# SenseBrain/JPD-SE

Hardware: AMD Instinct MI355X
Metric: training images/sec at 1024x512 (G+D+VGG step) (higher is better)
Workload: dtype bf16; 1 GPU; JPD-SE train step 1024x512, netG=global ngf=64 (39-ch input), num_D=2, VGG19+feat+L1, Adam x2, batch 4/GPU; global_batch=4, parallelism=dp1

## Files before the change

jpd-se_amd/csrc/conv_dispatch_fwd.h:

```cpp
#pragma once

namespace jpdse {

struct FwdCall {
  const jpdse_conv_desc* d; const ConvPlan& p;
  const void* x; const void* pack; const float* bias; void* y; void* ws; hipStream_t s;
  float* mom; void* pool; bool* pooled;
};

static int fwd_thin_in_rows(const FwdCall& c) {
  ThinInArgs g = {};
  g.DY = reinterpret_cast<const bf16_t*>(c.x);
  g.P = reinterpret_cast<const bf16_t*>(c.pack);
  g.DX = reinterpret_cast<bf16_t*>(c.y);
  g.bias = c.bias;
  g.act = c.d->act; g.slope = c.d->slope;
  g.N = c.d->N; g.H = c.d->H; g.W = c.d->W; g.OH = c.p.OH; g.OW = c.p.OW;
  g.py = g.px = 1;
  return launch_thin_in_rows<3, false>(g, c.s);
}

static int thin_fwd_slots(const ConvPlan& p, const ThinFwdGeom& tg) {
  return (p.OH % tg.TH == 0 && p.OW % tg.TW == 0) ? (p.OH / tg.TH) * (p.OW / tg.TW) : 0;
}
// ... 37 lines not shown
  HeadFwdArgs h = {};
  h.X = reinterpret_cast<const bf16_t*>(c.x);
  h.Wp = reinterpret_cast<const bf16_t*>(c.pack);
  h.bias = c.bias;
  h.Y = reinterpret_cast<bf16_t*>(c.y);
  h.N = d->N; h.H = d->H; h.W = d->W; h.OH = p.OH; h.OW = p.OW;
  h.K = d->K; h.Ks_out = p.Ks;
  h.R = d->R; h.S = d->S; h.pad = d->pad;
  h.reflect = d->pad_mode == JPDSE_PAD_REFLECT;
  h.act = d->act; h.slope = d->slope;
  h.tiles_w = (p.OW + 63) / 64;
  h.tiles_h = (p.OH + kHeadTH - 1) / kHeadTH;
  if (route == FwdRoute::head_rows) return p.Cs == 64 ? launch_head_rows<7>(h, c.s) : launch_head_rows<7, 32>(h, c.s);
  return p.Cs == 64 ? launch_head_fwd<64>(h, c.s) : launch_head_fwd<32>(h, c.s);
}

static int fwd_tapsum(const FwdCall& c) {
  const jpdse_conv_desc* d = c.d;
  const ConvPlan& p = c.p;
  const int cols = d->K * d->R * d->S, zs = (cols + 7) / 8 * 8;
  FastArgs f = {};
  f.X = reinterpret_cast<const bf16_t*>(c.x);
  f.B = reinterpret_cast<const bf16_t*>(c.pack);
  f.M = d->N * d->H * d->W; f.OH = f.IH = d->H; f.OW = f.IW = d->W;
  f.Cs = p.Cs; f.R = f.S = 1; f.sy = f.sx = 1;
  f.Kout = f.b_rows = cols; f.Ks = zs;
  f.act = JPDSE_ACT_NONE;
  f.splits = 1; f.no_finish = 1; f.partial = reinterpret_cast<float*>(c.ws);
  if (int rc = launch_fast(f, c.s)) return rc;
  const long long total = (long long)d->N * p.OH * p.OW * p.Ks;
  hipLaunchKernelGGL(tapsum_kernel, dim3((unsigned)((total + 255) / 256)), dim3(256), 0, c.s, f.partial, c.bias,
                     reinterpret_cast<bf16_t*>(c.y), d->N, d->H, d->W, p.OH, p.OW, d->K, p.Ks, d->R, d->S, d->pad,
                     d->pad_mode == JPDSE_PAD_REFLECT ? 1 : 0, zs, d->act, d->slope, total);
  return check_launch("tapsum_kernel");
}

static ConvView fwd_view(const FwdCall& c) {
  ConvView v = view_fwd(c.d, c.p, c.x, c.pack, c.bias, c.y);
  v.mom = c.mom;
  return v;
}
static float* splitk_slabs(const ConvPlan& p, void* ws) { return reinterpret_cast<float*>(reinterpret_cast<char*>(ws) + p.splitk_off); }

static int fwd_halo(const FwdCall& c) {
  HaloArgs h = to_halo(fwd_view(c));
  if (c.pool != nullptr && c.mom == nullptr && c.pooled != nullptr) {
    h.pool = reinterpret_cast<bf16_t*>(c.pool);
    *c.pooled = true;
  }
  return c.p.Ks > 64 ? launch_halo_cfg<2>(h, c.s) : launch_halo_cfg<1>(h, c.s);
}

static int fwd_fast(const FwdCall& c) {
  FastArgs f = to_fast(fwd_view(c));
  f.splits = splitk_for(f.M, c.p.Ks, c.d->R * c.d->S * c.p.Cs / 64);
  f.partial = splitk_slabs(c.p, c.ws);
  return launch_fast(f, c.s);
}

template <typename T>
static int fwd_gemm(const FwdCall& c, bool toep) {
  const jpdse_conv_desc* d = c.d;
  const ConvPlan& p = c.p;
  if (int rc = launch_pad<T>(c.x, c.ws, d->N, d->H, d->W, p.Cs, d->pad, d->pad, d->pad, d->pad, d->pad_mode, c.s)) return rc;
  const int px = toep ? 4 : 1, Lk = toep ? p.Lk_toep : p.Lk_fwd;
  GemmFwdArgs a = {};
  a.A = c.ws;
  a.B = toep ? reinterpret_cast<const char*>(c.pack) + p.fwd_pack_plain_bytes : c.pack;
  a.bias = c.bias;
  a.Y = c.y;
  a.OH = p.OH; a.OW = p.OW / px; a.M = d->N * a.OH * a.OW;
  a.Kout = toep ? 32 : d->K; a.Ks = a.b_rows = toep ? 32 : p.Ks;
  a.R = d->R; a.cpr = Lk / p.BKE; a.b_row_stride = (long long)d->R * Lk;
  a.in_sn = (long long)p.Hp * p.Wp * p.Cs; a.in_sr = (long long)p.Wp * p.Cs;
  a.in_sh = (long long)d->stride * p.Wp * p.Cs;
  a.in_sw = (long long)px * d->stride * p.Cs;
  a.out_sn = (long long)p.OH * p.OW * p.Ks; a.out_sh = (long long)p.OW * p.Ks; a.out_sw = (long long)px * p.Ks;
  a.act = d->act; a.slope = d->slope;
  if (toep) {
    a.col_mod = 8;
    a.k_real = d->K;
  } else {
    a.partial = splitk_slabs(p, c.ws);
    a.partial_cap = p.splitk_bytes;
  }
  return launch_fwd<T>(a, c.s);
}

template <typename T>
static int conv_fwd_t(const jpdse_conv_desc* d, const ConvPlan& p, const void* x, const void* pack,
                      const float* bias, void* y, void* ws, hipStream_t s, float* mom = nullptr, void* pool = nullptr,
                      bool* pooled = nullptr) {
  const FwdCall c = {d, p, x, pack, bias, y, ws, s, mom, pool, pooled};
  const FwdRoute route = select_fwd(d, p, {mom != nullptr, pool != nullptr});
  if constexpr (sizeof(T) == 2) {
    switch (route) {
      case FwdRoute::thin_in_rows: return fwd_thin_in_rows(c);
      case FwdRoute::thin_rows:
      case FwdRoute::thin_fwd: return fwd_thin(c, route);
      case FwdRoute::head_rows:
      case FwdRoute::head_fwd: return fwd_head(c, route);
      case FwdRoute::tapsum: return fwd_tapsum(c);
      case FwdRoute::rows: return launch_rows(to_rows(fwd_view(c)), d->stride, s);
      case FwdRoute::taps4: return launch_taps4(fwd_view(c), ws, s);
      case FwdRoute::taps9: return launch_taps9(fwd_view(c), splitk_slabs(p, ws), s);
      case FwdRoute::halo: return fwd_halo(c);
// ... 21 lines not shown
```

jpd-se_amd/csrc/conv_gemm.hip:

```cpp
#include "common.h"

#include <vector>


namespace jpdse {

struct GemmFwdArgs {
  const void* A;
  const void* B;
  const float* bias;
  void* Y;
  int M, OH, OW;
  int Kout, Ks;
  int R, cpr;
  int b_rows;
  long long b_row_stride;
  long long in_sn, in_sh, in_sw, in_sr, in_base;
  long long out_sn, out_sh, out_sw, out_base;
  int act;
  float slope;
  int col_mod, k_real;
  int splits;
  float* partial;
  size_t partial_cap;
// ... 93 lines not shown
  if (threadIdx.x == 0) reinterpret_cast<volatile int*>(occ_smem)[0] = (int)blockIdx.x;
  const unsigned long long t0 = __builtin_amdgcn_s_memrealtime();
  while (true) {
    const int r = __hip_atomic_load(release, __ATOMIC_RELAXED, __HIP_MEMORY_SCOPE_SYSTEM);
    if (r != 0) break;
    if (__builtin_amdgcn_s_memrealtime() - t0 > max_ticks) break;
    __builtin_amdgcn_s_sleep(127);
  }
}

int jpdse_debug_occupy_cus(int32_t blocks, const int32_t* release_flag, int32_t max_ms, void* stream) {
  JPDSE_REQUIRE(blocks > 0 && blocks <= 128 && release_flag != nullptr && max_ms > 0 && max_ms <= 20000,
                "debug_occupy_cus: blocks in 1..128, a flag, max_ms in 1..20000");
  constexpr int lds = 160 * 1024;
  if (int rc = opt_in_lds<&occupy_cus_kernel>("occupy_cus", lds)) return rc;
  hipLaunchKernelGGL(occupy_cus_kernel, dim3(blocks), dim3(256), lds, as_stream(stream), release_flag,
                     (unsigned long long)max_ms * 100000ULL);
  return check_launch("occupy_cus_kernel");
}

int jpdse_debug_set_fast_path(int32_t enable) {
  if (enable == 19 || enable == 28 || enable == 42 || enable == 43 || (enable >= 50 && enable <= 54) || enable == 56 || enable == 61 ||
      (enable >= 100 && enable <= 199) || (enable >= 201 && enable <= 203) || (enable >= 210 && enable <= 225))
    return set_error(JPDSE_EINVAL, "debug_set_fast_path: mode %d is retired (its code path was removed; see include/jpdse_dev.h)", (int)enable);
  g_fast_enabled = enable != 0;
  g_halo_enabled = enable != 3;
  g_moments_fused = enable != 32 && enable != 6;
  g_ring_virt = enable != 40 && enable != 6;
  g_thin1_enabled = enable != 41 && enable != 6;
  g_taps9_enabled = enable != 38 && enable != 6;
  g_taps4_enabled = enable != 36 && enable != 6;
  g_taps_enabled = enable != 35 && enable != 6;
  g_rows_enabled = enable != 29 && enable != 3;
  g_wgrad_nine_enabled = enable != 4;
  g_wgrad_taps_enabled = enable != 12;
  g_ring_enabled = enable != 7 && enable != 3;
  g_merge_min_kt = enable == 9 ? 16 : 4;
  g_norm_fused = enable != 27;
  g_merge_min_tiles = enable == 26 ? 384 : 64;
  g_fast_small = enable == 10 ? 0 : 20;
  g_halo_xcd = enable == 15 ? 1 : (enable == 16 ? 2 : (enable == 17 ? 3 : 0));
  g_halo_single = enable != 8;
  g_head_fwd_enabled = enable != 14 && enable != 6;
  g_thin_fwd_enabled = enable != 18;
  g_tapsum_enabled = enable != 13;
  g_thin_out_fast = enable != 13;
  g_toep_enabled = enable != 5;
  g_wgrad_nine32_enabled = enable != 55;
  g_head_rows32 = enable != 57;
  g_halo_xcd_auto = enable != 60;
  g_fast_fill = enable != 59;
  g_wgrad_taps_xcd = enable == 58;
  g_generic_splitk = enable != 48;
  g_splitk_enabled = enable != 6;
  return JPDSE_OK;
}

int jpdse_debug_conv_route(const jpdse_conv_desc* d, int32_t flags, int32_t out[3]) {
  if (int rc = validate(d)) return rc;
  JPDSE_REQUIRE(out != nullptr && (flags & ~0x7f) == 0, "debug_conv_route: null output or unknown flag bits");
  ConvPlan p;
  make_plan(d, &p);
  out[0] = (int32_t)select_fwd(d, p, {(flags & 1) != 0, (flags & 2) != 0});
  out[1] = (int32_t)select_dgrad(d, p, {(flags & 4) != 0, (flags & 8) != 0, (flags & 4) != 0 && (flags & 16) != 0, (flags & 32) != 0, (flags & 64) != 0});
  out[2] = (int32_t)select_wgrad(d, p);
  return JPDSE_OK;
}

const char* jpdse_debug_route_name(int32_t direction, int32_t route) {
  if (route < 0) return nullptr;
  if (direction == 0 && route <= (int)FwdRoute::generic) return route_name((FwdRoute)route);
  if (direction == 1 && route <= (int)DgradRoute::generic) return route_name((DgradRoute)route);
  if (direction == 2 && route <= (int)WgradRoute::generic) return route_name((WgradRoute)route);
  return nullptr;
}
#endif

int jpdse_prof_select(int32_t enable, int32_t Ks, int64_t kdim, int32_t max_launches) {
  g_prof.on = false;
  g_prof.used = 0;
  if (!enable) return JPDSE_OK;
  JPDSE_REQUIRE(Ks > 0 && kdim > 0 && max_launches > 0, "prof_select: bad selection");
  while ((int)g_prof.ev.size() < 2 * max_launches) {
    hipEvent_t e;
    if (hipEventCreate(&e) != hipSuccess) return set_error(JPDSE_ELAUNCH, "prof_select: hipEventCreate failed");
    g_prof.ev.push_back(e);
  }
  g_prof.flops.assign(max_launches, 0.0);
  g_prof.cls.assign(max_launches, 0);
  g_prof.Ks = Ks;
  g_prof.kdim = kdim;
  g_prof.on = true;
  return JPDSE_OK;
}

static int prof_sum(int cls, double* total_ms, double* total_flops, int64_t* launches) {
  double ms = 0.0, fl = 0.0;
  int64_t n = 0;
  for (int i = 0; i < g_prof.used; ++i) {
    if (g_prof.cls[i] != cls) continue;
    if (hipEventSynchronize(g_prof.ev[2 * i + 1]) != hipSuccess)
      return set_error(JPDSE_ELAUNCH, "prof_collect: hipEventSynchronize failed");
    float t = 0.f;
    if (hipEventElapsedTime(&t, g_prof.ev[2 * i], g_prof.ev[2 * i + 1]) != hipSuccess)
      return set_error(JPDSE_ELAUNCH, "prof_collect: hipEventElapsedTime failed");
    ms += t;
// ... 343 lines not shown
```

jpd-se_amd/csrc/conv_launch.h:

```cpp
#pragma once

namespace jpdse {

struct GemmProf {
  bool on = false;
  int Ks = 0;
  long long kdim = 0;
  int used = 0;
  std::vector<hipEvent_t> ev;
  std::vector<double> flops;
  std::vector<int> cls;
};
static GemmProf g_prof;
static int check_tile_grid(const char* who, int N, int OH, int OW, int th, int tw, int Cs_in, long long in_elems, long long out_elems) {
  if (N <= 0 || OH <= 0 || OW <= 0 || OH % th != 0 || OW % tw != 0)
    return set_error(JPDSE_EINVAL, "%s: output grid %d x %d x %d does not tile into %d x %d patches", who, N, OH, OW, th, tw);
  if (Cs_in <= 0 || Cs_in % 64 != 0) return set_error(JPDSE_EINVAL, "%s: %d input channels (a multiple of 64 is required)", who, Cs_in);
  if (in_elems >= (1LL << 31) || out_elems >= (1LL << 40))
    return set_error(JPDSE_EINVAL, "%s: tensor too large for the kernel's offsets (%lld input elements)", who, in_elems);
  return JPDSE_OK;
}

template <auto Kernel>
static int opt_in_lds(const char* who, int bytes) {
// ... 543 lines not shown
  a.mask = v.mask;
  a.prog[0].B[0] = v.B;
  a.prog[0].ktot[0] = v.ktot;
  a.prog[0].out_base[0] = v.out_base;
  for (int r = 0; r < v.R; ++r)
    for (int c = 0; c < v.S; ++c) {
      a.prog[0].tap_off[r * v.S + c] = r * patch_w + c;
      a.prog[0].tap_koff[r * v.S + c] = r * v.tap_r + c * v.tap_s;
    }
  return a;
}

static int launch_taps4(const ConvView& v, void* ws, hipStream_t s) {
  const int OHc = v.OH / 8 * 8, OWc = v.OW / 32 * 32;
  TapsArgs a = to_taps(v, 35);
  a.OH = OHc;
  a.OW = OWc;
  const int bn = v.Ks_out % 128 == 0 ? 128 : 64;
  a.nblk0 = v.N * (OHc / 8) * (OWc / 32) * ((v.Ks_out + bn - 1) / bn);
  if (int rc = bn == 128 ? launch_taps4_cfg<2>(a, a.nblk0, s) : launch_taps4_cfg<1>(a, a.nblk0, s)) return rc;
  const int k_tiles = 16 * v.Cin_s / 64;
  const int sp = taps4_fringe_splits(v.N, v.OH, v.OW, v.Ks_out, k_tiles);
  if (sp == 0) return JPDSE_OK;
  FastBatch fb = {};
  float* slab = reinterpret_cast<float*>(ws);
  const int rect[2][4] = {{OHc, 0, v.OH - OHc, v.OW}, {0, OWc, OHc, v.OW - OWc}};
  for (int q = 0; q < 2; ++q) {
    const int oh0 = rect[q][0], ow0 = rect[q][1], rows = rect[q][2], cols = rect[q][3];
    if (rows <= 0 || cols <= 0) continue;
    FastArgs g = to_fast(v);
    g.M = v.N * rows * cols;
    g.OH = rows;
    g.OW = cols;
    g.py = v.py - oh0;
    g.px = v.px - ow0;
    g.out_base = v.out_base + oh0 * v.out_sh + ow0 * v.out_sw;
    g.splits = sp;
    g.no_finish = 1;
    g.partial = slab;
    g.b_stride = v.ktot;
    g.b_tap_r = v.tap_r;
    g.b_tap_s = v.tap_s;
    slab += (size_t)sp * g.M * v.Ks_out;
    fb.p[fb.n++] = g;
  }
  if (int rc = launch_fast_batch(fb, s)) return rc;
  for (int q = 0; q < fb.n; ++q) {
    const long long total_vec = (long long)fb.p[q].M * (fb.p[q].Ks / 8);
    hipLaunchKernelGGL(splitk_finish_kernel, dim3(ew_blocks(total_vec)), dim3(256), 0, s, fb.p[q], total_vec);
  }
  return check_launch("taps4 fringe finish");
}

static int taps9_splits(int N, int OH, int OW, int Cin_s, int Ks_out) {
  const int sp = splitk_for(N * OH * OW, Ks_out, 9 * Cin_s / 64);
  const int cc = Cin_s / 64;
  return sp > cc / 2 ? (cc / 2 > 0 ? cc / 2 : 1) : sp;
}

template <int TN, bool VIRT = false>
static int launch_taps9_cfg(const TapsArgs& a, int total, hipStream_t s) {
  constexpr int PH = 10, PW = 34;
  constexpr int lds = 2 * ((PH * PW + 7) / 8) * 1024 + 3 * (2 * TN * 32) * 128;
  if (int rc = opt_in_lds<&gemm_taps_kernel<TN, 9, 0, 0, 0, 2, PH, PW, VIRT>>("gemm_taps(3x3)", lds)) return rc;
  if (int rc = check_tile_grid("gemm_taps(3x3)", a.N, a.OH, a.OW, 8, 32, a.Cs, (long long)a.N * a.IH * a.IW * a.Cs,
                               (long long)a.N * a.OH * a.OW * a.Ks)) return rc;
  const int sp = a.splits > 1 ? a.splits : 1;
  if (total != sp * a.N * (a.OH / 8) * (a.OW / 32) * ((a.Ks + 2 * TN * 32 - 1) / (2 * TN * 32)) || (sp > 1 && a.partial == nullptr))
    return set_error(JPDSE_EINVAL, "gemm_taps(3x3): %d blocks do not match the tile grid x %d splits", total, sp);
  if (VIRT && (a.V == nullptr || a.py != 1 || a.px != 1 || a.IH != a.OH || a.IW != a.OW || a.OH < 16 || a.reflect))
    return set_error(JPDSE_EINVAL, "gemm_taps(3x3): folded-frame form needs a frame, pad 1, equal grids, >= 16 rows");
  hipLaunchKernelGGL((gemm_taps_kernel<TN, 9, 0, 0, 0, 2, PH, PW, VIRT>), dim3(total), dim3(512), lds, s, a);
  return check_launch("gemm_taps_kernel(3x3)");
}

static int launch_taps9(const ConvView& v, float* slabs, hipStream_t s) {
  TapsArgs a = to_taps(v, 34);
  a.reflect = v.reflect;
  a.V = v.frame;
  const int bn = v.Ks_out % 128 == 0 ? 128 : 64;
  const int tiles = v.N * (v.OH / 8) * (v.OW / 32) * ((v.Ks_out + bn - 1) / bn);
  a.splits = taps9_splits(v.N, v.OH, v.OW, v.Cin_s, v.Ks_out);
  a.partial = a.splits > 1 ? slabs : nullptr;
  a.nblk0 = tiles * (a.splits > 1 ? a.splits : 1);
  int rc;
  if (v.frame != nullptr) rc = bn == 128 ? launch_taps9_cfg<2, true>(a, a.nblk0, s) : launch_taps9_cfg<1, true>(a, a.nblk0, s);
  else rc = bn == 128 ? launch_taps9_cfg<2>(a, a.nblk0, s) : launch_taps9_cfg<1>(a, a.nblk0, s);
  if (rc) return rc;
  if (a.splits <= 1) return JPDSE_OK;
  FastArgs f = {};
  f.Y = v.Y;
  f.bias = v.bias;
  f.M = v.N * v.OH * v.OW;
  f.OH = v.OH;
  f.OW = v.OW;
  f.Kout = v.Kout;
  f.Ks = v.Ks_out;
  f.out_sn = v.out_sn;
  f.out_sh = v.out_sh;
  f.out_sw = v.out_sw;
  f.out_base = v.out_base;
  f.act = v.act;
  f.slope = v.slope;
  f.splits = a.splits;
  f.partial = slabs;
  f.addend = v.addend;
// ... 53 lines not shown
```

jpd-se_amd/csrc/conv_route.h:

```cpp
#pragma once

namespace jpdse {

enum class FwdRoute { thin_in_rows, thin_rows, thin_fwd, head_rows, head_fwd, tapsum, rows, taps4, taps9, halo, fast, toeplitz, generic };
enum class DgradRoute { rows, halo, taps9, ring_taps9_frame, ring_halo_frame, ring_taps9_strips, ring_halo_strips, head, dgrad2_rows,
                        thin_dgrad2_rows, thin_in_rows, taps_dgrad2, taps4, thin1, fast, generic };
enum class WgradRoute { thin1, tap_expanded, taps, nine, head, thin, fast, generic };

static const char* const kFwdRouteNames[] = {"thin_in_rows", "thin_rows", "thin_fwd", "head_rows", "head_fwd", "tapsum", "rows",
                                             "taps4", "taps9", "halo", "fast", "toeplitz", "generic"};
static const char* const kDgradRouteNames[] = {"rows", "halo", "taps9", "ring_taps9_frame", "ring_halo_frame", "ring_taps9_strips",
                                               "ring_halo_strips", "head", "dgrad2_rows", "thin_dgrad2_rows", "thin_in_rows",
                                               "taps_dgrad2", "taps4", "thin1", "fast", "generic"};
static const char* const kWgradRouteNames[] = {"thin1", "tap_expanded", "taps", "nine", "head", "thin", "fast", "generic"};
static_assert(sizeof(kFwdRouteNames) / sizeof(char*) == (size_t)FwdRoute::generic + 1 &&
              sizeof(kDgradRouteNames) / sizeof(char*) == (size_t)DgradRoute::generic + 1 &&
              sizeof(kWgradRouteNames) / sizeof(char*) == (size_t)WgradRoute::generic + 1, "one name per route");
static const char* route_name(FwdRoute r) { return kFwdRouteNames[(int)r]; }
static const char* route_name(DgradRoute r) { return kDgradRouteNames[(int)r]; }
static const char* route_name(WgradRoute r) { return kWgradRouteNames[(int)r]; }

JPDSE_SWITCH(bool, g_fast_enabled, true);
JPDSE_SWITCH(int, g_toep_enabled, 1);
JPDSE_SWITCH(int, g_halo_enabled, 1);
JPDSE_SWITCH(int, g_halo_single, 1);
JPDSE_SWITCH(int, g_rows_enabled, 1);
JPDSE_SWITCH(int, g_head_rows32, 1);
JPDSE_SWITCH(int, g_thin_fwd_enabled, 1);
JPDSE_SWITCH(int, g_head_fwd_enabled, 1);
JPDSE_SWITCH(int, g_tapsum_enabled, 1);
JPDSE_SWITCH(int, g_taps_enabled, 1);
JPDSE_SWITCH(int, g_taps4_enabled, 1);
JPDSE_SWITCH(int, g_taps9_enabled, 1);
JPDSE_SWITCH(int, g_ring_enabled, 1);
JPDSE_SWITCH(int, g_ring_virt, 1);
JPDSE_SWITCH(int, g_merge_min_kt, 4);
JPDSE_SWITCH(int, g_merge_min_tiles, 64);
JPDSE_SWITCH(int, g_thin1_enabled, 1);
JPDSE_SWITCH(int, g_wgrad_taps_enabled, 1);
JPDSE_SWITCH(int, g_wgrad_nine_enabled, 1);
JPDSE_SWITCH(int, g_wgrad_nine32_enabled, 1);

struct ConvShape {
  int N, IH, IW, Cin_s, OH, OW;
  int R, S, stride, reflect;
  int act, Ks_out;
  int tap_r;
};
static ConvShape shape_fwd(const jpdse_conv_desc* d, const ConvPlan& p) {
  return {d->N, d->H, d->W, p.Cs, p.OH, p.OW, d->R, d->S, d->stride, d->pad_mode == JPDSE_PAD_REFLECT, d->act, p.Ks, p.Lk_fwd};
}
static ConvShape shape_dgrad_phase(const jpdse_conv_desc* d, const ConvPlan& p, int i) {
  const Phase& f = p.ph[i];
  return {d->N, p.OH, p.OW, p.Ks, f.cnth, f.cntw, f.Uh, f.Uw, 1, 0, JPDSE_ACT_NONE, p.Cs, f.Lk};
}

static bool rows_ok(const ConvShape& v) {
  return g_fast_enabled && g_rows_enabled && v.R == 3 && v.S == 3 && (v.stride == 1 || v.stride == 2) && !v.reflect && v.Cin_s == 64 &&
         v.Ks_out % 64 == 0 && v.OW % 64 == 0 && v.OH % 4 == 0 &&
         (v.act == JPDSE_ACT_NONE || v.act == JPDSE_ACT_RELU || v.act == JPDSE_ACT_LRELU);
}
static bool halo_ok(int R, int S, int stride, int OH, int OW, int Cs_in, int Ks_out) {
  return g_fast_enabled && g_halo_enabled && R == 3 && S == 3 && stride == 1 && OH % 4 == 0 && OW % 64 == 0 &&
         Cs_in % 64 == 0 && Ks_out > 32;
}
static bool halo_ok(const ConvShape& v) { return halo_ok(v.R, v.S, v.stride, v.OH, v.OW, v.Cin_s, v.Ks_out); }
static bool taps4_shape_ok(const ConvShape& v) {
  return v.tap_r == v.S * v.Cin_s && g_fast_enabled && g_taps4_enabled && v.R == 4 && v.S == 4 && v.stride == 1 && v.OH >= 8 && v.OW >= 32 &&
         v.Cin_s % 64 == 0 && v.Cin_s >= 128 && v.Ks_out % 64 == 0 && v.Ks_out >= 64 && (long long)v.N * v.IH * v.IW * v.Cin_s < (1LL << 31) &&
         (long long)v.Ks_out * 16 * v.Cin_s < (1LL << 31);
}
static bool taps9_shape_ok(int R, int S, int stride, int OH, int OW, int Cin_s, int Ks_out, long long x_elems, long long b_elems) {
  return g_fast_enabled && g_taps9_enabled && R == 3 && S == 3 && stride == 1 && OH % 8 == 0 && OW % 32 == 0 && OW % 64 != 0 &&
         Cin_s % 64 == 0 && Cin_s >= 128 && Ks_out % 64 == 0 && x_elems < (1LL << 31) && b_elems < (1LL << 31);
}
static bool taps9_shape_ok(const ConvShape& v) {
  return v.tap_r == v.S * v.Cin_s && taps9_shape_ok(v.R, v.S, v.stride, v.OH, v.OW, v.Cin_s, v.Ks_out, (long long)v.N * v.IH * v.IW * v.Cin_s,
                                                    (long long)v.Ks_out * 9 * v.Cin_s);
}

static bool thin_in_rows_fwd_ok(const jpdse_conv_desc* d, const ConvPlan& p) {
  return g_fast_enabled && g_rows_enabled && p.Cs == 8 && d->R == 3 && d->S == 3 && d->stride == 1 && d->pad == 1 &&
         d->pad_mode == JPDSE_PAD_ZERO && p.Ks == 64 && d->K == 64 && p.Lk_fwd == 32 &&
         (d->act == JPDSE_ACT_NONE || d->act == JPDSE_ACT_RELU || d->act == JPDSE_ACT_LRELU);
}
struct ThinFwdGeom { int TH, TW, strip_units, w_units, lds; };
static bool thin_fwd_geom(const jpdse_conv_desc* d, const ConvPlan& p, ThinFwdGeom* g) {
  if (!(g_fast_enabled && g_thin_fwd_enabled && p.thinf)) return false;
  const int st = d->stride;
  g->w_units = (p.Ks * p.KP_thin * 2 + 1023) / 1024;
  static const int cand[3][2] = {{8, 64}, {4, 64}, {4, 32}};
  for (int c = (p.Cs <= 8 && p.Ks == 64) ? 1 : 0; c < 3; ++c) {
    const int TH = cand[c][0], TW = cand[c][1];
    if (TH == 4 && p.Ks != 64) break;
    g->strip_units = (((TW - 1) * st + d->S) * p.Cs * 2 + 16 + 1023) / 1024;
    const int lds = (((TH - 1) * st + d->R) * g->strip_units + 2 * g->w_units) * 1024;
    const int epi = TH * TW * (p.Ks * 2 + 64);
    g->TH = TH;
    g->TW = TW;
    g->lds = lds > epi ? lds : epi;
    if (g->lds <= 160 * 1024) return true;
  }
  return false;
}
static bool thin_rows_ok(const jpdse_conv_desc* d, const ConvPlan& p) {
  return g_rows_enabled && d->stride == 2 && d->R == 4 && d->S == 4 && p.Cs == 40 && p.Ks == 64 && d->K == 64 &&
         d->pad_mode != JPDSE_PAD_REFLECT && p.KP_thin == 168 &&
         (d->act == JPDSE_ACT_NONE || d->act == JPDSE_ACT_RELU || d->act == JPDSE_ACT_LRELU);
}
static bool head_fwd_ok(const jpdse_conv_desc* d, const ConvPlan& p) {
  const int ncols = d->K * d->R * d->S;
  return g_fast_enabled && g_head_fwd_enabled && p.ES == 2 && d->stride == 1 && d->K <= 3 && p.Ks == 8 &&
         (p.Cs == 64 || p.Cs == 32) && d->R == 7 && d->S == 7 && ncols <= 160 && p.Lk_fwd == d->S * p.Cs;
}
static bool head_rows_ok(int cin, int R, int K, int Ks_out, int H, int W, int OH, int OW) {
  return g_rows_enabled && (cin == 64 || (cin == 32 && g_head_rows32 && R == 7)) && K <= 3 && Ks_out == 8 && OW % 128 == 0 &&
         OH % 8 == 0 && OH == H && OW == W;
}
static bool tapsum_ok(const jpdse_conv_desc* d, const ConvPlan& p) {
  return g_fast_enabled && g_tapsum_enabled && p.ES == 2 && d->stride == 1 && d->K * d->R * d->S <= 32 &&
         p.Cs % 64 == 0 && p.Cs >= 256 && p.Lk_fwd == d->S * p.Cs;
}

static bool prefer_320(int M, int Ks) {
  if (Ks <= 64) return false;
  const long long nt = (Ks + 127) / 128;
  const long long t256 = (long long)((M + 255) / 256) * nt, t320 = (long long)((M + 319) / 320) * nt;
  const long long c256 = ((t256 + 255) / 256) * 256, c320 = ((t320 + 255) / 256) * 320;
  return c320 < c256;
}
static bool fast_pays(int M, int Ks, int k_tiles) {
  if (!g_fast_enabled) return false;
  if (k_tiles < 8) return false;
  if (Ks <= 32) {
    if (!(g_thin_out_fast && k_tiles >= 64)) return false;
    return splitk_for(M, Ks, k_tiles) > 1 || (M + 255) / 256 >= 128;
  }
  if (splitk_for(M, Ks, k_tiles) > 1) return true;
  const int bn = Ks > 64 ? 128 : (Ks > 32 ? 64 : 32);
  const long long tiles = (long long)((M + 255) / 256) * ((Ks + bn - 1) / bn);
  if (prefer_320(M, Ks)) {
    const long long t320 = (long long)((M + 319) / 320) * ((Ks + 127) / 128);
    if (t320 % 256 == 0 || t320 % 256 >= 192 || t320 >= 448) return true;
  }
  return tiles >= 448 || (tiles >= 256 && tiles % 256 == 0);
}

struct FwdWants { bool mom, pool; };
static FwdRoute select_fwd(const jpdse_conv_desc* d, const ConvPlan& p, FwdWants w) {
  if (d->dtype == JPDSE_BF16) {
    if (thin_in_rows_fwd_ok(d, p)) return FwdRoute::thin_in_rows;
    ThinFwdGeom tg;
    if (thin_fwd_geom(d, p, &tg)) return thin_rows_ok(d, p) ? FwdRoute::thin_rows : FwdRoute::thin_fwd;
    if (head_fwd_ok(d, p)) return head_rows_ok(p.Cs, d->R, d->K, p.Ks, d->H, d->W, p.OH, p.OW) ? FwdRoute::head_rows : FwdRoute::head_fwd;
    if (tapsum_ok(d, p)) return FwdRoute::tapsum;
    const ConvShape v = shape_fwd(d, p);
    if (rows_ok(v)) return FwdRoute::rows;
    if (!v.reflect && !w.mom && taps4_shape_ok(v)) return FwdRoute::taps4;
    if (!w.mom && taps9_shape_ok(v)) return FwdRoute::taps9;
    if (halo_ok(v)) return FwdRoute::halo;
    if (p.Cs % 64 == 0 && fast_pays(d->N * p.OH * p.OW, p.Ks, d->R * d->S * p.Cs / 64)) return FwdRoute::fast;
  }
  return p.toep && g_fast_enabled && g_toep_enabled && p.OW % 4 == 0 ? FwdRoute::toeplitz : FwdRoute::generic;
}

struct TapsDgrad2Geom { int core_h, core_w; };
static bool taps_dgrad2_geom(const jpdse_conv_desc* d, const ConvPlan& p, bool mom, TapsDgrad2Geom* g) {
  if (!(g_fast_enabled && g_taps_enabled) || d->dtype != JPDSE_BF16 || d->pad_mode == JPDSE_PAD_REFLECT) return false;
  if (d->stride != 2 || d->R != 3 || d->S != 3 || d->pad != 1 || p.nph != 4) return false;
  if (mom) return false;
  if (p.Ks % 64 != 0 || p.Ks < 128 || p.Cs % 64 != 0) return false;
  if ((long long)d->N * p.OH * p.OW * p.Ks >= (1LL << 31) || (long long)p.Cs * 4 * p.Ks >= (1LL << 31)) return false;
  const int core_h = p.ph[0].cnth, core_w = p.ph[0].cntw;
  if (core_h < 4 || core_h % 4 != 0 || core_w < 64 || core_w % 64 != 0) return false;
  for (int i = 0; i < 4; ++i) {
    const Phase& f = p.ph[i];
    if (f.Lk != f.Uw * p.Ks) return false;
    if (f.Uh != (f.qh == 0 ? 2 : 1) || f.Uw != (f.qw == 0 ? 2 : 1)) return false;
    if ((f.Uh - 1) - f.i0h != 0 || (f.Uw - 1) - f.i0w != 0) return false;
    if (f.cnth != core_h || f.cntw != core_w) return false;
  }
  if (g != nullptr) *g = {core_h, core_w};
  return true;
}
static bool taps_dgrad2_ok(const jpdse_conv_desc* d, const ConvPlan& p, bool mom) { return taps_dgrad2_geom(d, p, mom, nullptr); }

static bool thin1_shape_ok(const jpdse_conv_desc* d, int Cs, int Ks) {
  const int cv = Cs >> 3;
  return g_fast_enabled && g_thin1_enabled && d->dtype == JPDSE_BF16 && d->K == 1 && Ks == 8 && d->stride == 1 &&
         d->pad_mode != JPDSE_PAD_REFLECT && d->R == 4 && d->S == 4 && d->pad <= 3 && Cs % 128 == 0 && d->C == Cs &&
         cv <= 256 && (cv & (cv - 1)) == 0;
}

static int live_phases(const ConvPlan& p) {
  int n = 0;
  for (int i = 0; i < p.nph; ++i) n += p.ph[i].cnth > 0 && p.ph[i].cntw > 0;
  return n;
}
static bool dgrad_fast_pays(const jpdse_conv_desc* d, const ConvPlan& p) {
  if (p.Ks % 64 != 0) return false;
  long long tiles = 0;
  int kt_max = 0, m_single = 0;
  const int bn = p.Cs > 64 ? 128 : (p.Cs > 32 ? 64 : 32);
  for (int i = 0; i < p.nph; ++i) {
    if (p.ph[i].cnth <= 0 || p.ph[i].cntw <= 0) continue;
    const int Mi = d->N * p.ph[i].cnth * p.ph[i].cntw;
    tiles += (long long)((Mi + 255) / 256) * ((p.Cs + bn - 1) / bn);
    const int kt = p.ph[i].Uh * p.ph[i].Uw * p.Ks / 64;
    kt_max = kt > kt_max ? kt : kt_max;
    m_single = Mi;
  }
  if (live_phases(p) == 1) return fast_pays(m_single, p.Cs, kt_max);
  return g_fast_enabled && p.Cs > 32 && kt_max >= g_merge_min_kt && tiles >= g_merge_min_tiles;
}
// ... 84 lines not shown
```

jpd-se_amd/csrc/gemm_taps.h:

```cpp
#pragma once
#include "common.h"
#include "gemm_fast.h"
#include "gemm_halo.h"

namespace jpdse {

constexpr int kTapsMax = 16;

struct TapsProg {
  const bf16_t* B[2];
  long long ktot[2];
  long long out_base[2];
  int tap_off[kTapsMax];
  int tap_koff[kTapsMax];
};

struct TapsArgs {
  const bf16_t* X;
  bf16_t* Y;
  const float* bias;
  int N, OH, OW;
  int IH, IW, Cs;
  int py, px;
  int Kout, Ks, b_rows;
  long long out_sn, out_sh, out_sw;
  int act;
  float slope;
  const bf16_t* addend;
  const bf16_t* mask;
  float mask_slope;
  int reflect;
  int splits;
  float* partial;
  const bf16_t* V;
  int nblk0;
  TapsProg prog[2];
};

template <int TN, int T0, int T1, int WROWS, int PH, int PW, bool VIRT = false>
__device__ __forceinline__ void gemm_taps_body(const TapsArgs& a, const TapsProg& pr, int bid, char* smem) {
  constexpr int NT = T0 + T1, NSETS = T1 > 0 ? 2 : 1;
  constexpr int NW = 8, WN = 2;
  constexpr int TH = 4 * WROWS, TW = 64 / WROWS;
  constexpr int BN = WN * TN * 32;
  constexpr int NP = PH * PW;
  constexpr int UH = (NP + 7) / 8;
  constexpr int HALO = UH * 1024;
  constexpr int B_STAGE = BN * 128;
  constexpr int B_UNITS = BN / 8, BU = B_UNITS / NW;
  static_assert(B_UNITS % NW == 0, "every wave issues exactly BU weight pieces per tile");
  constexpr int HU = (UH + NW - 1) / NW;
  constexpr int UPT = (HU + NT - 1) / NT;
  static_assert(NT <= kTapsMax && NT >= 2, "tap program length");
  constexpr int PZ = UH * 8 - 1;
  static_assert(!VIRT || (T0 == 9 && T1 == 0 && PZ - 1 >= NP && (PZ & 1) == 1 && (PW & 1) == 0 && PH == TH + 2 && PW == TW + 2), "VIRT: nine taps, one set, two slack pixels");
  char* const bring = smem;
  char* const halo0 = smem + 3 * B_STAGE;

  const int tid = threadIdx.x, lane = tid & 63;
  const int wid = __builtin_amdgcn_readfirstlane(tid >> 6);
  const int wm = wid / WN, wn = wid % WN;
  const int tiles_w = a.OW / TW, tiles_h = a.OH / TH;
  const int tiles_m = a.N * tiles_h * tiles_w;
  const int ntiles = tiles_m * ((a.Ks + BN - 1) / BN);
  const int split = a.splits > 1 ? bid / ntiles : 0;
  if (a.splits > 1) bid -= split * ntiles;
  const int tile_m = bid % tiles_m, tile_n = bid / tiles_m;
  const int tw_i = tile_m % tiles_w, t1 = tile_m / tiles_w;
  const int th_i = t1 % tiles_h, n = t1 / tiles_h;
  const int oh0 = th_i * TH, ow0 = tw_i * TW, n0 = tile_n * BN;
  const int lrow = lane >> 3, lslot = lane & 7;
  const bf16_t* const zero = reinterpret_cast<const bf16_t*>(g_zero_page);

  int h_off[HU];
  int h_lds[HU];
  int n_hu = 0;
#pragma unroll
  for (int i = 0; i < HU; ++i) {
    const int u = wid + i * NW;
    const bool on = u < UH;
    n_hu += on ? 1 : 0;
    const int ug = on ? u : 0;
    int p = ug * 8 + lrow;
    const int swz_p = p;
    const bool slack = p >= NP;
    p = p < NP ? p : NP - 1;
    const int hr = p / PW, wc = p - hr * PW;
    int ih = oh0 - a.py + hr, iw = ow0 - a.px + wc;
    bool ok = ((unsigned)ih < (unsigned)a.IH) & ((unsigned)iw < (unsigned)a.IW);
    if (a.reflect) {
      ih = ih < 0 ? -ih : (ih >= a.IH ? 2 * (a.IH - 1) - ih : ih);
      iw = iw < 0 ? -iw : (iw >= a.IW ? 2 * (a.IW - 1) - iw : iw);
      ok = ((unsigned)ih < (unsigned)a.IH) & ((unsigned)iw < (unsigned)a.IW);
    }
    const int chunk = (lslot ^ (swz_p >> 1)) & 7;
    h_off[i] = ok ? ((n * a.IH + ih) * a.IW + iw) * a.Cs + chunk * 8 : -1;
    if constexpr (VIRT) {
      if (!ok && !slack) {
        const int fw = a.IW + 2;
        const bool both = ow0 == 0 && ow0 + TW == a.IW;
        const bool colf = iw < 0 || iw >= a.IW;
        const int iws = (both && colf) ? (iw < 0 ? a.IW : -1) : iw;
        const int fp = (ih < 0 || ih >= a.IH) ? (ih < 0 ? 0 : fw) + iws + 1 : 2 * fw + (iws < 0 ? 0 : a.IH) + ih;
        const int cls = iws < 0 ? hr * PW + 3 : (iws >= a.IW ? hr * PW + TW - 2 : swz_p);
        const int chunk_v = (lslot ^ (cls >> 1)) & 7;
        h_off[i] = -2 - ((n * (2 * fw + 2 * a.IH) + fp) * a.Cs + chunk_v * 8);
      }
      if (slack) h_off[i] = -1;
    }
    h_lds[i] = ug * 1024;
  }
  int b_off[NSETS][BU];
  int b_lds[BU];
#pragma unroll
  for (int j = 0; j < BU; ++j) {
    const int u = wid + j * NW;
    const int row = u * 8 + lrow;
    int br = n0 + row;
    br = br < a.b_rows ? br : a.b_rows - 1;
#pragma unroll
    for (int q = 0; q < NSETS; ++q) b_off[q][j] = br * (int)pr.ktot[q] + ((lslot ^ (row >> 1)) & 7) * 8;
    b_lds[j] = u * 1024;
  }

  const int CC_all = a.Cs >> 6;
  const int s_begin = a.splits > 1 ? CC_all * split / a.splits : 0;
  const int CC = a.splits > 1 ? CC_all * (split + 1) / a.splits : CC_all;

  auto issue_patch_unit = [&](int i, int slab) {
    char* const dst = halo0 + (slab & 1) * HALO + h_lds[i];
    const bf16_t* src = h_off[i] >= 0 ? a.X + (h_off[i] + slab * 64) : zero;
    if constexpr (VIRT) src = h_off[i] < -1 ? a.V + ((-2 - h_off[i]) + slab * 64) : src;
    glds16(src, dst);
  };
  auto issue_b = [&](const int tap, const int slab, const int stage) {
    const int q = tap < T0 ? 0 : 1;
    char* const st = bring + stage * B_STAGE;
    const bf16_t* const base = pr.B[q] + (pr.tap_koff[tap] + slab * 64);
#pragma unroll
    for (int j = 0; j < BU; ++j) glds16(base + b_off[q][j], st + b_lds[j]);
  };

#pragma unroll
  for (int i = 0; i < HU; ++i)
    if (i < n_hu) issue_patch_unit(i, s_begin);
  issue_b(0, s_begin, 0);
  issue_b(1, s_begin, 1);

  int pb[2];
#pragma unroll
  for (int i = 0; i < 2; ++i)
    pb[i] = WROWS == 1 ? wm * PW + i * 32 + (lane & 31) : (2 * wm + i) * PW + (lane & 31);
  int vc0 = 0, vc2 = 0;
  bool v_top = false, v_bot = false;
  if constexpr (VIRT) {
    static_assert(!VIRT || WROWS == 2, "VIRT is written for the 8 x 32 tile (one fragment block per image row)");
    v_top = oh0 == 0;
    v_bot = oh0 + TH == a.OH;
    const bool left = ow0 == 0, right = ow0 + TW == a.OW;
    const int w = lane & 31;
    vc0 = (left && w == 0) ? 1000 : ((right && w == TW - 2) ? (left ? 0 : PW - 1) : w);
    vc2 = (right && w == TW - 1) ? 1000 : ((left && w == 1) ? (right ? PW - 1 : 0) : w + 2);
  }
  const int hsel = lane >> 5;
  int b_rd[TN][4];
#pragma unroll
  for (int j = 0; j < TN; ++j) {
    const int row = wn * TN * 32 + j * 32 + (lane & 31);
#pragma unroll
    for (int ks = 0; ks < 4; ++ks) b_rd[j][ks] = swz128(row, 2 * ks + hsel);
  }

  f32x16 acc[NSETS][2][TN];
#pragma unroll
  for (int q = 0; q < NSETS; ++q)
#pragma unroll
    for (int i = 0; i < 2; ++i)
#pragma unroll
      for (int j = 0; j < TN; ++j)
#pragma unroll
        for (int e = 0; e < 16; ++e) acc[q][i][j][e] = 0.f;

  auto step = [&](const int SM, const int TAP, const int slab, const bool more, const char* const hb) {
    if (TAP < NT - 1 || more) wait_vmcnt<BU>(); else wait_vmcnt<0>();
    __builtin_amdgcn_s_barrier();
    if (more) {
#pragma unroll
      for (int i = 0; i < HU; ++i)
        if (i >= TAP * UPT && i < (TAP + 1) * UPT && i < n_hu) issue_patch_unit(i, slab + 1);
    }
    {
// ... 44 lines not shown
    __builtin_amdgcn_s_setprio(0);
  };

  for (int slab0 = s_begin; slab0 < CC; slab0 += 3) {
#pragma unroll
    for (int sm = 0; sm < 3; ++sm) {
      const int slab = slab0 + sm;
      if (slab >= CC) break;
      const bool more = slab + 1 < CC;
      const char* const hb = halo0 + (slab & 1) * HALO;
#pragma unroll
      for (int tap = 0; tap < NT; ++tap) step(sm, tap, slab, more, hb);
    }
  }

  if (a.splits > 1) {
    float* const slab = a.partial + (long long)split * ((long long)a.N * a.OH * a.OW) * a.Ks;
#pragma unroll
    for (int j = 0; j < TN; ++j) {
      const int col = n0 + wn * TN * 32 + j * 32 + (lane & 31);
      if (col >= a.Ks) continue;
#pragma unroll
      for (int i = 0; i < 2; ++i) {
#pragma unroll
        for (int e = 0; e < 16; ++e) {
          const int rl = i * 32 + (e & 3) + 8 * (e >> 2) + 4 * (lane >> 5);
          const int r = WROWS == 1 ? wm : 2 * wm + (rl >> 5), c = WROWS == 1 ? rl : (rl & 31);
          const long long m = ((long long)n * a.OH + oh0 + r) * a.OW + ow0 + c;
          slab[m * a.Ks + col] = acc[0][i][j][e];
        }
      }
    }
    return;
  }
  constexpr int PITCH = BN * 2 + 64;
  static_assert(TH * TW * PITCH <= 2 * HALO + 3 * B_STAGE, "epilogue tile fits the pipeline LDS");
  constexpr int VPR = BN / 8;
#pragma unroll
  for (int q = 0; q < NSETS; ++q) {
    __syncthreads();
    acc_tile_to_lds<2, TN>(smem, PITCH, WROWS == 1 ? wm * 64 : wm * 64, wn * TN * 32, n0, lane, acc[q], a.bias, a.Kout, a.act, a.slope);
    __syncthreads();
    const long long blk_base = pr.out_base[q] + n * a.out_sn + (long long)oh0 * a.out_sh + (long long)ow0 * a.out_sw;
    if (a.addend != nullptr || a.mask != nullptr) {
      constexpr int NV = TH * TW * VPR / 512;
      static_assert(TH * TW * VPR % 512 == 0, "every thread owns the same number of output vectors");
      u32x4 addv[NV], mskv[NV];
#pragma unroll
      for (int it = 0; it < NV; ++it) {
        const int idx = tid + 512 * it;
        const int row = idx / VPR, v = idx - row * VPR;
        const int r = row / TW, c = row - r * TW;
        const long long off = blk_base + (long long)r * a.out_sh + (long long)c * a.out_sw + n0 + v * 8;
        const bool on = n0 + v * 8 < a.Ks;
        if (on && a.addend != nullptr) addv[it] = *reinterpret_cast<const u32x4*>(a.addend + off);
        if (on && a.mask != nullptr) mskv[it] = *reinterpret_cast<const u32x4*>(a.mask + off);
      }
#pragma unroll
      for (int it = 0; it < NV; ++it) {
        const int idx = tid + 512 * it;
        const int row = idx / VPR, v = idx - row * VPR;
        if (n0 + v * 8 >= a.Ks) continue;
        const int r = row / TW, c = row - r * TW;
        const long long off = blk_base + (long long)r * a.out_sh + (long long)c * a.out_sw + n0 + v * 8;
        u32x4 val = *reinterpret_cast<const u32x4*>(smem + row * PITCH + v * 16);
        if (a.addend != nullptr) val = add_bf16x8(val, addv[it]);
        if (a.mask != nullptr) val = lrelu_mask8(val, mskv[it], a.mask_slope);
        *reinterpret_cast<u32x4*>(a.Y + off) = val;
      }
      continue;
    }
    for (int idx = tid; idx < TH * TW * VPR; idx += 512) {
      const int row = idx / VPR, v = idx - row * VPR;
      if (n0 + v * 8 >= a.Ks) continue;
      const int r = row / TW, c = row - r * TW;
      const long long off = blk_base + (long long)r * a.out_sh + (long long)c * a.out_sw;
      *reinterpret_cast<u32x4*>(a.Y + off + n0 + v * 8) = *reinterpret_cast<const u32x4*>(smem + row * PITCH + v * 16);
    }
  }
}

template <int TN, int T0A, int T1A, int T0B, int T1B, int WROWS, int PH, int PW, bool VIRT = false>
__global__ __launch_bounds__(512) void gemm_taps_kernel(const TapsArgs a) {
  extern __shared__ __attribute__((aligned(16))) char smem[];
  if constexpr (T0B > 0) {
    const int b = (int)blockIdx.x;
    int prog, local;
    if ((a.nblk0 & 7) == 0) {
      prog = (b >> 3) & 1;
      local = ((b >> 4) << 3) | (b & 7);
    } else {
      prog = b >= a.nblk0 ? 1 : 0;
      local = prog ? b - a.nblk0 : b;
    }
    if (prog) {
      gemm_taps_body<TN, T0B, T1B, WROWS, PH, PW>(a, a.prog[1], local, smem);
      return;
    }
    gemm_taps_body<TN, T0A, T1A, WROWS, PH, PW>(a, a.prog[0], local, smem);
  } else {
    gemm_taps_body<TN, T0A, T1A, WROWS, PH, PW, VIRT>(a, a.prog[0], (int)blockIdx.x, smem);
  }
}

}
```

Measured before the change: 156.2 images/sec.

## Route 4x4 stride-2 pad-2 forward convs through a space-to-depth pair taps kernel

Adds a PAIR mode to the taps GEMM kernel that treats a 4x4 stride-2 conv as a 2x2 stride-1 conv over 2x2 pixel pairs. The halo tile is loaded once and reused across four taps, with sub-pixel channel slabs. This is meant to replace the im2col-style fast GEMM path for the discriminator downsampling layers. A block-count heuristic picks the 8x32 tile form and otherwise falls back to the fast path. Ragged output tiles are masked in the epilogue, which adds bounds checks and per-pixel validity bits.

```diff
diff --git a/jpd-se_amd/csrc/conv_dispatch_fwd.h b/jpd-se_amd/csrc/conv_dispatch_fwd.h
--- a/jpd-se_amd/csrc/conv_dispatch_fwd.h
+++ b/jpd-se_amd/csrc/conv_dispatch_fwd.h
@@ -113,6 +113,7 @@
 }
 
 static int fwd_fast(const FwdCall& c) {
+  if (const ConvView v = fwd_view(c); pair_fwd_form(v, c.d->pad)) return launch_taps_pair(v, pair_fwd_form(v, c.d->pad), c.s);
   FastArgs f = to_fast(fwd_view(c));
   f.splits = splitk_for(f.M, c.p.Ks, c.d->R * c.d->S * c.p.Cs / 64);
   f.partial = splitk_slabs(c.p, c.ws);
diff --git a/jpd-se_amd/csrc/conv_gemm.hip b/jpd-se_amd/csrc/conv_gemm.hip
--- a/jpd-se_amd/csrc/conv_gemm.hip
+++ b/jpd-se_amd/csrc/conv_gemm.hip
@@ -169,6 +169,7 @@
   g_fast_fill = enable != 59;
   g_wgrad_taps_xcd = enable == 58;
   g_generic_splitk = enable != 48;
+  g_pairview = enable == 62 || enable == 63 ? enable : (enable == 64 || enable == 6 ? 0 : 1);
   g_splitk_enabled = enable != 6;
   return JPDSE_OK;
 }
diff --git a/jpd-se_amd/csrc/conv_launch.h b/jpd-se_amd/csrc/conv_launch.h
--- a/jpd-se_amd/csrc/conv_launch.h
+++ b/jpd-se_amd/csrc/conv_launch.h
@@ -619,6 +619,43 @@
   return check_launch("taps4 fringe finish");
 }
 
+template <int TN, int WROWS>
+static int launch_taps_pair_cfg(const TapsArgs& a, int total, hipStream_t s) {
+  constexpr int TH = 4 * WROWS, TW = 64 / WROWS, PH = TH + 1, PW = TW + 1;
+  constexpr int lds = 2 * ((PH * PW + 7) / 8) * 1024 + 3 * (2 * TN * 32) * 128;
+  static_assert(lds >= TH * TW * (2 * TN * 32 * 2 + 64) && lds <= 160 * 1024, "pipeline LDS holds the epilogue tile");
+  if (int rc = opt_in_lds<&gemm_taps_kernel<TN, 4, 0, 0, 0, WROWS, PH, PW, false, true>>("gemm_taps(pair)", lds)) return rc;
+  if (a.N <= 0 || a.OH != a.IH / 2 + 1 || a.OW != a.IW / 2 + 1 || a.py != 1 || a.px != 1 || a.Cs < 64 || a.Cs != (64 << a.pair_csh) ||
+      a.pair_tap_r != 4 * a.Cs || a.splits > 1 || a.reflect || (long long)a.N * a.IH * a.IW * a.Cs >= (1LL << 31) ||
+      16LL * a.Cs * a.b_rows >= (1LL << 31))
+    return set_error(JPDSE_EINVAL, "gemm_taps(pair): not a 4x4 stride-2 pad-2 layer of 64 * 2^j input channels");
+  if (total != a.N * ((a.OH + TH - 1) / TH) * ((a.OW + TW - 1) / TW) * ((a.Ks + 2 * TN * 32 - 1) / (2 * TN * 32)))
+    return set_error(JPDSE_EINVAL, "gemm_taps(pair): %d blocks do not match the tile grid", total);
+  hipLaunchKernelGGL((gemm_taps_kernel<TN, 4, 0, 0, 0, WROWS, PH, PW, false, true>), dim3(total), dim3(512), lds, s, a);
+  return check_launch("gemm_taps_kernel(pair)");
+}
+
+static int launch_taps_pair(const ConvView& v, int form, hipStream_t s) {
+  const int wrows = form == 63 ? 2 : 1, th = 4 * wrows, tw = 64 / wrows;
+  TapsArgs a = to_taps(v, tw + 1);
+  a.py = a.px = 1;
+  a.pair_csh = __builtin_ctz(v.Cin_s / 64);
+  a.pair_tap_r = v.tap_r;
+  for (int r = 0; r < 2; ++r)
+    for (int c = 0; c < 2; ++c) {
+      a.prog[0].tap_off[r * 2 + c] = r * (tw + 1) + c;
+      a.prog[0].tap_koff[r * 2 + c] = 2 * r * v.tap_r + 2 * c * v.tap_s;
+    }
+  const int bn = v.Ks_out % 128 == 0 ? 128 : 64;
+  a.nblk0 = v.N * ((v.OH + th - 1) / th) * ((v.OW + tw - 1) / tw) * ((v.Ks_out + bn - 1) / bn);
+  const int pslot = prof_begin(s, v.Ks_out, 16LL * v.Cin_s);
+  int rc;
+  if (wrows == 2) rc = bn == 128 ? launch_taps_pair_cfg<2, 2>(a, a.nblk0, s) : launch_taps_pair_cfg<1, 2>(a, a.nblk0, s);
+  else rc = bn == 128 ? launch_taps_pair_cfg<2, 1>(a, a.nblk0, s) : launch_taps_pair_cfg<1, 1>(a, a.nblk0, s);
+  prof_end(pslot, 0, 2.0 * (double)v.N * v.OH * v.OW * (double)v.Ks_out * 16.0 * (double)v.Cin_s, s);
+  return rc;
+}
+
 static int taps9_splits(int N, int OH, int OW, int Cin_s, int Ks_out) {
   const int sp = splitk_for(N * OH * OW, Ks_out, 9 * Cin_s / 64);
   const int cc = Cin_s / 64;
diff --git a/jpd-se_amd/csrc/conv_route.h b/jpd-se_amd/csrc/conv_route.h
--- a/jpd-se_amd/csrc/conv_route.h
+++ b/jpd-se_amd/csrc/conv_route.h
@@ -70,6 +70,20 @@
          v.Cin_s % 64 == 0 && v.Cin_s >= 128 && v.Ks_out % 64 == 0 && v.Ks_out >= 64 && (long long)v.N * v.IH * v.IW * v.Cin_s < (1LL << 31) &&
          (long long)v.Ks_out * 16 * v.Cin_s < (1LL << 31);
 }
+JPDSE_SWITCH(int, g_pairview, 1);
+static bool pair_shape_ok(const ConvShape& v, int pad) {
+  return g_fast_enabled && v.R == 4 && v.S == 4 && v.stride == 2 && pad == 2 && !v.reflect && v.Cin_s >= 64 &&
+         v.Cin_s <= 512 && (v.Cin_s & (v.Cin_s - 1)) == 0 && v.Ks_out % 64 == 0 && v.tap_r == v.S * v.Cin_s &&
+         (long long)v.N * v.IH * v.IW * v.Cin_s < (1LL << 31) && v.OH == v.IH / 2 + 1 && v.OW == v.IW / 2 + 1;
+}
+static bool pair_forced(const ConvShape& v, int pad) { return g_pairview >= 62 && pair_shape_ok(v, pad); }
+static int pair_fwd_form(const ConvShape& v, int pad) {
+  if (!pair_shape_ok(v, pad) || g_pairview == 0) return 0;
+  if (g_pairview >= 62) return g_pairview;
+  const long long blocks = (long long)v.N * ((v.OH + 7) / 8) * ((v.OW + 31) / 32) * ((v.Ks_out + 127) / 128);
+  const long long rounds = (blocks + 255) / 256;
+  return (blocks <= 256 || 4 * blocks >= 3 * 256 * rounds) ? 63 : 0;
+}
 static bool taps9_shape_ok(int R, int S, int stride, int OH, int OW, int Cin_s, int Ks_out, long long x_elems, long long b_elems) {
   return g_fast_enabled && g_taps9_enabled && R == 3 && S == 3 && stride == 1 && OH % 8 == 0 && OW % 32 == 0 && OW % 64 != 0 &&
          Cin_s % 64 == 0 && Cin_s >= 128 && Ks_out % 64 == 0 && x_elems < (1LL << 31) && b_elems < (1LL << 31);
@@ -159,7 +173,7 @@
     if (!v.reflect && !w.mom && taps4_shape_ok(v)) return FwdRoute::taps4;
     if (!w.mom && taps9_shape_ok(v)) return FwdRoute::taps9;
     if (halo_ok(v)) return FwdRoute::halo;
-    if (p.Cs % 64 == 0 && fast_pays(d->N * p.OH * p.OW, p.Ks, d->R * d->S * p.Cs / 64)) return FwdRoute::fast;
+    if (p.Cs % 64 == 0 && (pair_forced(v, d->pad) || fast_pays(d->N * p.OH * p.OW, p.Ks, d->R * d->S * p.Cs / 64))) return FwdRoute::fast;
   }
   return p.toep && g_fast_enabled && g_toep_enabled && p.OW % 4 == 0 ? FwdRoute::toeplitz : FwdRoute::generic;
 }
diff --git a/jpd-se_amd/csrc/gemm_taps.h b/jpd-se_amd/csrc/gemm_taps.h
--- a/jpd-se_amd/csrc/gemm_taps.h
+++ b/jpd-se_amd/csrc/gemm_taps.h
@@ -34,10 +34,11 @@
   float* partial;
   const bf16_t* V;
   int nblk0;
+  int pair_csh, pair_tap_r;
   TapsProg prog[2];
 };
 
-template <int TN, int T0, int T1, int WROWS, int PH, int PW, bool VIRT = false>
+template <int TN, int T0, int T1, int WROWS, int PH, int PW, bool VIRT = false, bool PAIR = false>
 __device__ __forceinline__ void gemm_taps_body(const TapsArgs& a, const TapsProg& pr, int bid, char* smem) {
   constexpr int NT = T0 + T1, NSETS = T1 > 0 ? 2 : 1;
   constexpr int NW = 8, WN = 2;
@@ -53,6 +54,7 @@
   constexpr int UPT = (HU + NT - 1) / NT;
   static_assert(NT <= kTapsMax && NT >= 2, "tap program length");
   constexpr int PZ = UH * 8 - 1;
+  static_assert(!PAIR || (!VIRT && T0 == 4 && T1 == 0 && PH == TH + 1 && PW == TW + 1), "PAIR: four taps, one set");
   static_assert(!VIRT || (T0 == 9 && T1 == 0 && PZ - 1 >= NP && (PZ & 1) == 1 && (PW & 1) == 0 && PH == TH + 2 && PW == TW + 2), "VIRT: nine taps, one set, two slack pixels");
   char* const bring = smem;
   char* const halo0 = smem + 3 * B_STAGE;
@@ -60,7 +62,7 @@
   const int tid = threadIdx.x, lane = tid & 63;
   const int wid = __builtin_amdgcn_readfirstlane(tid >> 6);
   const int wm = wid / WN, wn = wid % WN;
-  const int tiles_w = a.OW / TW, tiles_h = a.OH / TH;
+  const int tiles_w = PAIR ? (a.OW + TW - 1) / TW : a.OW / TW, tiles_h = PAIR ? (a.OH + TH - 1) / TH : a.OH / TH;
   const int tiles_m = a.N * tiles_h * tiles_w;
   const int ntiles = tiles_m * ((a.Ks + BN - 1) / BN);
   const int split = a.splits > 1 ? bid / ntiles : 0;
@@ -74,6 +76,7 @@
 
   int h_off[HU];
   int h_lds[HU];
+  int h_ok[HU];
   int n_hu = 0;
 #pragma unroll
   for (int i = 0; i < HU; ++i) {
@@ -95,6 +98,13 @@
     }
     const int chunk = (lslot ^ (swz_p >> 1)) & 7;
     h_off[i] = ok ? ((n * a.IH + ih) * a.IW + iw) * a.Cs + chunk * 8 : -1;
+    if constexpr (PAIR) {
+      const int ih0 = 2 * ih, iw0 = 2 * iw;
+      const int okh = ((unsigned)ih0 < (unsigned)a.IH ? 1 : 0) | ((unsigned)(ih0 + 1) < (unsigned)a.IH ? 2 : 0);
+      const int okw = ((unsigned)iw0 < (unsigned)a.IW ? 1 : 0) | ((unsigned)(iw0 + 1) < (unsigned)a.IW ? 2 : 0);
+      h_ok[i] = ((okh & 1) ? okw : 0) | ((okh & 2) ? okw << 2 : 0);
+      h_off[i] = ((n * a.IH + ih0) * a.IW + iw0) * a.Cs + chunk * 8;
+    }
     if constexpr (VIRT) {
       if (!ok && !slack) {
         const int fw = a.IW + 2;
@@ -123,7 +133,7 @@
     b_lds[j] = u * 1024;
   }
 
-  const int CC_all = a.Cs >> 6;
+  const int CC_all = PAIR ? 4 * (a.Cs >> 6) : a.Cs >> 6;
   const int s_begin = a.splits > 1 ? CC_all * split / a.splits : 0;
   const int CC = a.splits > 1 ? CC_all * (split + 1) / a.splits : CC_all;
 
@@ -131,12 +141,18 @@
     char* const dst = halo0 + (slab & 1) * HALO + h_lds[i];
     const bf16_t* src = h_off[i] >= 0 ? a.X + (h_off[i] + slab * 64) : zero;
     if constexpr (VIRT) src = h_off[i] < -1 ? a.V + ((-2 - h_off[i]) + slab * 64) : src;
+    if constexpr (PAIR) {
+      const int sub = slab >> a.pair_csh, cs = slab & ((1 << a.pair_csh) - 1);
+      const int xo = ((sub >> 1) * a.IW + (sub & 1)) * a.Cs + cs * 64;
+      src = ((h_ok[i] >> sub) & 1) ? a.X + (h_off[i] + xo) : zero;
+    }
     glds16(src, dst);
   };
   auto issue_b = [&](const int tap, const int slab, const int stage) {
     const int q = tap < T0 ? 0 : 1;
     char* const st = bring + stage * B_STAGE;
-    const bf16_t* const base = pr.B[q] + (pr.tap_koff[tap] + slab * 64);
+    const int slab_koff = PAIR ? (slab >> (a.pair_csh + 1)) * a.pair_tap_r + (slab & ((2 << a.pair_csh) - 1)) * 64 : slab * 64;
+    const bf16_t* const base = pr.B[q] + (pr.tap_koff[tap] + slab_koff);
 #pragma unroll
     for (int j = 0; j < BU; ++j) glds16(base + b_off[q][j], st + b_lds[j]);
   };
@@ -287,7 +303,7 @@
         const int row = idx / VPR, v = idx - row * VPR;
         const int r = row / TW, c = row - r * TW;
         const long long off = blk_base + (long long)r * a.out_sh + (long long)c * a.out_sw + n0 + v * 8;
-        const bool on = n0 + v * 8 < a.Ks;
+        const bool on = n0 + v * 8 < a.Ks && (!PAIR || (oh0 + r < a.OH && ow0 + c < a.OW));
         if (on && a.addend != nullptr) addv[it] = *reinterpret_cast<const u32x4*>(a.addend + off);
         if (on && a.mask != nullptr) mskv[it] = *reinterpret_cast<const u32x4*>(a.mask + off);
       }
@@ -297,6 +313,7 @@
         const int row = idx / VPR, v = idx - row * VPR;
         if (n0 + v * 8 >= a.Ks) continue;
         const int r = row / TW, c = row - r * TW;
+        if (PAIR && (oh0 + r >= a.OH || ow0 + c >= a.OW)) continue;
         const long long off = blk_base + (long long)r * a.out_sh + (long long)c * a.out_sw + n0 + v * 8;
         u32x4 val = *reinterpret_cast<const u32x4*>(smem + row * PITCH + v * 16);
         if (a.addend != nullptr) val = add_bf16x8(val, addv[it]);
@@ -309,13 +326,14 @@
       const int row = idx / VPR, v = idx - row * VPR;
       if (n0 + v * 8 >= a.Ks) continue;
       const int r = row / TW, c = row - r * TW;
+      if (PAIR && (oh0 + r >= a.OH || ow0 + c >= a.OW)) continue;
       const long long off = blk_base + (long long)r * a.out_sh + (long long)c * a.out_sw;
       *reinterpret_cast<u32x4*>(a.Y + off + n0 + v * 8) = *reinterpret_cast<const u32x4*>(smem + row * PITCH + v * 16);
     }
   }
 }
 
-template <int TN, int T0A, int T1A, int T0B, int T1B, int WROWS, int PH, int PW, bool VIRT = false>
+template <int TN, int T0A, int T1A, int T0B, int T1B, int WROWS, int PH, int PW, bool VIRT = false, bool PAIR = false>
 __global__ __launch_bounds__(512) void gemm_taps_kernel(const TapsArgs a) {
   extern __shared__ __attribute__((aligned(16))) char smem[];
   if constexpr (T0B > 0) {
@@ -334,7 +352,7 @@
     }
     gemm_taps_body<TN, T0A, T1A, WROWS, PH, PW>(a, a.prog[0], local, smem);
   } else {
-    gemm_taps_body<TN, T0A, T1A, WROWS, PH, PW, VIRT>(a, a.prog[0], (int)blockIdx.x, smem);
+    gemm_taps_body<TN, T0A, T1A, WROWS, PH, PW, VIRT, PAIR>(a, a.prog[0], (int)blockIdx.x, smem);
   }
 }
 
```

Measured after the change: 156.3 images/sec, median of 3. About the same (+0.1%).
